# 10XGenomics/scan-rs

Hardware: AMD Instinct MI355X
Metric: cells/sec for top-50 PCA on 1000000x33000 @3% nnz; achieved HBM GB/s vs roofline (higher is better)
Workload: dtype f64

## Files before the change

### scan-rs_amd/csrc/capi.cpp

```cpp
#include <algorithm>
#include <cmath>
#include <vector>

#include "common.hpp"
#include "col_moments_plan.hpp"
#include "bk_plan.hpp"
#include "spmm_route.hpp"
#include "shard_exchange.hpp"

namespace scanrs {

static void allreduce_any(Storage &st, void *d, uint64_t count, int dtype) {
    if (!st.shard.active()) return;
    if (st.prof.on) st.prof.begin(st.stream, dtype == 0 ? "allreduce_f64" : "allreduce_u64", (double)count * 8.0);
    if (st.shard.comm) {
        comm_allreduce(st, st.shard.comm, d, count, dtype);
    } else if (st.shard.allreduce) {
        SCANRS_SYNC(st.stream);
        if (st.shard.allreduce(st.shard.ctx, d, count, dtype) != 0) fail(SCANRS_ERR_DEVICE, "all-reduce callback failed");
    } else {
        fail(SCANRS_ERR_ARGUMENT, "sharded handle without a transport");
    }
    if (st.prof.on) st.prof.end(st.stream);
}
// ... 1409 lines not shown
            st.device_factor = value != 0.0;
        } else if (k == "sseq_grid_cap") {
            st.sseq_grid_cap = as_u32(1, 16384);
        } else if (k == "merge_fused") {
            st.merge_fused = (int)as_u32(0, 1);
        } else if (k == "subset_scatter") {
            st.subset_scatter = (int)as_u32(0, 1);
        } else if (k == "d2h_threads") {
            st.d2h_threads = as_u32(1, 256);
        } else if (k == "sync_timeout_s") {
            set_sync_timeout_checked(value);
        } else if (k == "tile_spare_cus") {
            st.tile_spare_cus = value != 0.0;
        } else if (k == "tile_poison_slack") {
            st.tile_poison_slack = value != 0.0;
        } else if (k == "spmv_row_table") {
            st.spmv_row_table = value != 0.0;
        } else if (k == "gemm_direct") {
            st.gemm_direct = value != 0.0;
        } else if (k == "reuse_cmax") {
            if (!(value > 0.0)) fail(SCANRS_ERR_ARGUMENT, "reuse_cmax must be positive");
            st.reuse_cmax = value;
        } else {
            fail(SCANRS_ERR_ARGUMENT, "unknown option '%s'", key);
        }
    });
}
int scanrs_mat_get_counter(scanrs_mat *m, const char *key, uint64_t *value) {
    return guard([&] {
        if (!m || !key || !value) fail(SCANRS_ERR_ARGUMENT, "null argument");
// ... 17 lines not shown
                *value = d.flagged_older;
            else if (k == "bk_limit_branch")
                *value = d.limit_branch;
            else if (k == "bk_limit_bits")
                *value = bits(d.limit);
            else if (k == "bk_direct_columns")
                *value = d.direct_columns;
            else if (k == "bk_last_direct")
                *value = d.last_direct;
            else if (k == "bk_full_direct")
                *value = d.full_direct;
            else if (k == "bk_early_projections")
                *value = d.early_projections;
            else if (k == "bk_cmax_dense_bits")
                *value = bits(d.cmax_dense);
            else
                fail(SCANRS_ERR_ARGUMENT, "unknown counter '%s'", key);
        } else if (k == "spmm_route")
            *value = m->st->spmm.family;
        else if (k == "spmm_form")
            *value = m->st->spmm.form;
        else if (k == "spmm_chunks")
            *value = m->st->spmm.chunks;
        else if (k == "partition_rounds")
            *value = m->st->partition_rounds;
        else if (k == "partition_allreduces")
            *value = m->st->partition_allreduces;
        else if (k == "de_pairs_passes")
            *value = m->st->de_pairs_passes;
        else if (k == "de_pairs_literal")
            *value = m->st->de_pairs_literal;
        else if (k == "de_shard_tests")
            *value = m->st->de_shard_tests;
        else if (k == "de_shard_allreduces")
            *value = m->st->de_shard_allreduces;
        else if (k == "subset_masked_passes")
// ... 318 lines not shown
```

### scan-rs_amd/csrc/common.hpp

```cpp
#pragma once
#include <atomic>
#include <chrono>
#include <condition_variable>
#include <cstring>
#include <cstdio>
#include <cstdint>
#include <cstdarg>
#include <functional>
#include <map>
#include <set>
#include <memory>
#include <mutex>
#include <new>
#include <string>
#include <thread>
#include <utility>
#include <vector>

#include <hip/hip_runtime.h>

#include "scanrs_amd.h"
#include "common_err.hpp"

struct scanrs_comm;
// ... 326 lines not shown
    uint32_t sseq_grid_cap = 16384;
    int merge_fused = 1;
    size_t l2_tile_bytes = 3584u << 10;
    int spmm_order = 1;
    uint32_t hot_segment = 512;
    uint64_t blocked_min_nnz = 1ull << 22;
    int slice_walk = 1;
    int spmv_lds = 1;
    int dense_side_no_lds = 0;
    int overlap = 1;
    const int *skip_flag = nullptr;
    uint64_t orth_fallbacks = 0;
    uint64_t bk_host_retries = 0;
    struct BkDecisions {
        uint64_t q = 0, b = 0, coef_valid = 0, flagged_older = 0, limit_branch = 0, direct_columns = 0, last_direct = 0, full_direct = 0,
                 early_projections = 0;
        double limit = 0.0, cmax_dense = 0.0;
    } bk;
    int col_moments = 1;
    int device_factor = 1;
    unsigned d2h_threads = 4;
    int tile_poison_slack = 0;
    int tile_spare_cus = 1;
    int spmv_row_table = 1;
    int gemm_direct = 1;
    double reuse_cmax = 1e5;
    int materialize = 1;
    struct SpmmDecision {
        uint64_t family = 0, form = 0, chunks = 0;
    } spmm;
    ~Storage();
    SparseCopy &copy_with_outer_rows(bool outer_rows);
};
struct Storage::SideBuild {
    std::thread th;
    hipStream_t stream = nullptr;
    const SparseCopy *order[2] = {nullptr, nullptr};
    bool want_layout[2] = {false, false};
// ... 429 lines not shown
```

### scan-rs_amd/csrc/kernels.hip

```cpp
#include "common.hpp"
#include "device_map.hpp"
#include "spmm_route.hpp"
#include "launch_util.hpp"

#include <algorithm>
#include <rocprim/rocprim.hpp>

namespace scanrs {

template <typename T>
struct Vec2;
template <>
struct Vec2<double> {
    typedef d2 type;
};
template <>
struct Vec2<uint32_t> {
    typedef u2 type;
};

template <typename T>
__device__ __forceinline__ T bcast(T v, uint32_t lane);
template <>
__device__ __forceinline__ double bcast<double>(double v, uint32_t lane) {
// ... 1276 lines not shown
        hipLaunchKernelGGL((slab_reduce_kernel<double, 1>), dim3((cp.n_multi + 3u) / 4u), block, 0, st.stream, cp.multi.p, cp.n_multi,
                           slab, l, out, ldo, off_a, rank, off_w, ldw);
    SCANRS_HIP(hipGetLastError());
}

void launch_spmm_f64(Storage &st, SparseCopy &cp, const DevMap &map, const double *X, uint32_t ldx, uint32_t l,
                     double *out, uint32_t ldo, const double *off_a, uint32_t rank, const double *off_w, uint32_t ldw) {
    SpmmQuery q = spmm_query(st, cp, map, l, ldx);
    const bool tiles = tiles_static_candidate(q) && (path_forces_tiles(q.o) || spmm_tiles_auto(st, cp, map));
    SpmmRoute r = spmm_route(q, tiles);
    if (r.materialized && !fvals_room(cp)) {
        q.values_room = false;
        r = spmm_route(q, tiles);
    }
    st.spmm = {(uint64_t)r.family, r.form_bits(), r.chunk_bits()};
    if (r.even_ld && ((ldx & 1u) || (ldo & 1u))) fail(SCANRS_ERR_ARGUMENT, "panel leading dimensions must be even");
    const double *fv = r.materialized ? ensure_fvals(st, cp, map, r.fstart) : nullptr;
    switch (r.family) {
    case SPMM_TILES:
        for (uint32_t c0 = 0; c0 < l; c0 += r.chunk_width) {
            const uint32_t lw = std::min(r.chunk_width, l - c0);
            if (r.sliver && c0 + lw == l)
                launch_spmm_t<double>(st, cp, map, X + c0, ldx, lw, out + c0, ldo, off_a, rank, off_w ? off_w + c0 : nullptr, ldw);
            else
                launch_spmm_tiles(st, cp, map, X + c0, ldx, lw, out + c0, ldo, off_a, rank, off_w ? off_w + c0 : nullptr, ldw);
        }
        return;
    case SPMM_GATHER2D: return launch_spmm_2d(st, cp, map, X, ldx, l, out, ldo, off_a, rank, off_w, ldw);
    case SPMM_GATHER2D_F32: return launch_spmm_2d_f32(st, cp, map, X, ldx, l, out, ldo, off_a, rank, off_w, ldw);
    case SPMM_SLICE_WALK:
// ... 118 lines not shown
```

### scan-rs_amd/csrc/solver.cpp

```cpp
#include <algorithm>
#include <atomic>
#include <cmath>
#include <cstdlib>
#include <cstring>
#include <future>
#include <sys/mman.h>
#include <memory>
#include <mutex>
#include <thread>
#include <vector>

#include "bk_plan.hpp"
#include "common.hpp"
#include "host_team.hpp"

namespace scanrs {

struct SmallRng {
    uint64_t s[4];
    explicit SmallRng(uint64_t seed) {
        uint64_t state = seed;
        for (int i = 0; i < 4; i++) {
            state += 0x9E3779B97F4A7C15ull;
            uint64_t z = state;
// ... 1123 lines not shown
            for (uint32_t r = 0; r < q; r++)
                for (uint32_t j = 0; j < q; j++) colmax[j] = std::max(colmax[j], std::fabs(cfull[(size_t)r * q + j]));
        if (reuse && !c_valid && trace_on())
            fprintf(stderr, "[scanrs trace] bk: rank-deficient panels were completed on the host: the projection is computed directly\n");
        plan = bk_plan(colmax.data(), b, n_iter, c.st.reuse_cmax, c_valid);
        bk_record(c.st.bk, plan, c_valid);
        if (tracked && trace_on()) bk_plan_trace(colmax.data(), b, n_iter, plan);
        if (tracked && !plan.last_direct) {
            Tick tk("bk: last block product");
            mat_apply(m, to_t_transpose, P, ldb, b, T + (size_t)(n_iter - 1) * b, ldq);
        }
    }

    const double *project() {
        Tick tk("bk: projection");
        if (plan.full_direct) {
            wait_early_projections();
            mat_apply(m, to_t_transpose, K, ldq, q, T, ldq);
        } else {
            for (uint32_t j = n_iter - 1 - (plan.last_direct ? 1u : 0u); j >= 1; j--)
                if (!projected[j]) project_block(c, j, "bk_projw");
            if (!block0_copied) launch_copy_cols(c.st, T, ldq, T2, ldq, dt, b);
            wait_early_projections();
            if (!plan.direct.empty()) {
                const uint32_t nbad = (uint32_t)plan.direct.size(), ldbad = even_up(nbad);
                uint32_t *d_idx = c.st.scratch.get<uint32_t>("bk_badidx", nbad);
                SCANRS_HIP(hipMemcpyAsync(d_idx, plan.direct.data(), (size_t)nbad * 4, hipMemcpyHostToDevice, c.s));
                c.sync();
                double *Qbad = c.dev("bk_Qbad", (size_t)ds * ldbad);
                double *Tbad = c.dev("bk_Tbad", (size_t)dt * ldbad);
                launch_permute_cols(c.st, K, ldq, Qbad, ldbad, ds, d_idx, nbad, false);
                mat_apply(m, to_t_transpose, Qbad, ldbad, nbad, Tbad, ldbad);
                launch_permute_cols(c.st, Tbad, ldbad, T2, ldq, dt, d_idx, nbad, true);
            }
        }
        stage_mark("bk projection sync");
        c.sync();
        stage_mark("bk projection synced");
        return plan.full_direct ? T : T2;
// ... 285 lines not shown
```

### scan-rs_amd/csrc/tiles.hip

```cpp
#include "common.hpp"
#include "device_map.hpp"
#include "spmm_route.hpp"

#include <algorithm>
#include <rocprim/rocprim.hpp>

namespace scanrs {

namespace {

#ifndef TL_NW_DEF
#define TL_NW_DEF 8
#endif
constexpr uint32_t TL_NW = TL_NW_DEF;
constexpr int TL_W = 6;
#ifndef TL_SROWS
#define TL_SROWS 1
#endif
#ifndef TL_DPPW
#define TL_DPPW 1
#endif
typedef uint32_t u32x16 __attribute__((ext_vector_type(16)));
constexpr uint32_t TL_TABC = 8;

// ... 676 lines not shown
    DevBuf<double> uo, vi;
    DevBuf<double> uo_slot;
    DevBuf<double> ratio_tab;
    bool dense = false;
    uint32_t dn_wgg = 0, dn_items = 0;
    uint64_t dn_chunks = 0;
    uint64_t dn_served = 0;
    uint64_t src_nnz = 0;
    DevBuf<uint32_t> drec;
    DevBuf<uint64_t> cmeta;
    DevBuf<char> ditems;
    DevBuf<uint32_t> rtab;
    int slot_mode = 0;
    DevBuf<uint32_t> slot_order;
    DevBuf<uint32_t> slot_pos;
    DevBuf<double> w_place, w_inner;
    bool fold_inner = false, fold_outer = false;
    bool separable = false;
    int wsrc = 0;
    DevBuf<double> wtab;
    uint64_t wtab_stride = 0;
    int sig_n = -1;
    uint32_t sig_id[MAX_OPS] = {};
    int sig_outer[MAX_OPS] = {};
    double bytes() const {
        return (double)prow.n * 2.0 + (double)pcnt.n + (double)pw.n * 8.0 + (double)ov.nnz * 16.0 + (double)ratio_tab.n * 8.0 + (double)drec.n * 4.0 + (double)cmeta.n * 8.0 +
               (double)rtab.n * 4.0 + (double)wtab.n * 8.0 + (double)(w_place.n + w_inner.n) * 8.0;
    }
    bool structure_matches(const Storage &st) const {
        if (dense != tile_dense_wanted(st)) return false;
        if (dense && (slot_order.n != 0) != (st.tile_sort_slots != 0 && n_slots > 1)) return false;
        if (dense && slot_order.n != 0 && slot_mode != st.tile_sort_slots) return false;
        const bool splittable = default_tile_shape(spmm_options(st));
        const double want_x = splittable && st.tile_split ? st.tile_split_x : 0.0, want_min = splittable && st.tile_split ? st.tile_split_min : 0.0;
        return sh.K == st.tile_k && sh.S == st.tile_s && sh.T == st.tile_t && sh.B == st.tile_b && sh.KU == tile_unit_positions(spmm_options(st)) &&
               split_x == want_x && split_min == want_min;
    }
    bool weights_match(const DevMap &map) const {
        if (sig_n != map.n) return false;
        for (int i = 0; i < map.n; i++)
            if (sig_id[i] != map.ops[i].id || sig_outer[i] != map.ops[i].a_outer) return false;
        return true;
// ... 268 lines not shown
        } else
        hipLaunchKernelGGL(tile_weights_kernel, grid, dim3(256), 0, st.stream, tl.prow.p, tl.pcnt.p, tl.pw.p, n_rec,
                           tl.slot_vec.p, tl.n_slots, tl.sh, map, tl.unit_mode ? tl.uo.p : (const double *)nullptr, tl.unit_mode ? tl.vi.p : (const double *)nullptr, skip,
                           tl.unit_mode ? tl.ratio_tab.p : (const double *)nullptr, nl_outer, vmajor ? (uint32_t)tl.n_groups : 0u);
    }
    if (tl.ov.nnz) materialize_map_values(st, tl.ov, map, tl.ov.fvals.p);
    SCANRS_HIP(hipGetLastError());
    if (trace_on()) (void)wait_stream_quiet(st.stream);
    tl.sig_n = map.n;
    for (int i = 0; i < map.n; i++) {
        tl.sig_id[i] = map.ops[i].id;
        tl.sig_outer[i] = map.ops[i].a_outer;
    }
}

#include "tiles_dense.inc"

namespace {

struct TileArgs {
    const uint16_t *prow;
    const double *pw;
    const double *uo;
    uint32_t *next_item;
    uint64_t n_groups, n_outer, n_inner;
    TileShape sh;
};

template <int K, int S, int KU>
__device__ __forceinline__ void spmm_tile_body(const TileArgs &ta, const double *__restrict__ X, uint32_t ldx, uint32_t l,
// ... 217 lines not shown
                                                                  uint32_t n_items) {
    spmm_tile_body<K, S, KU>(ta, X, ldx, l, parts, ldo, part_stride, n_items);
}
template <int K, int S, int KU>
__global__ __launch_bounds__(64 * TL_NW) __attribute__((amdgpu_waves_per_eu(3, 3))) void spmm_tile_kernel_r168(
    TileArgs ta, const double *__restrict__ X, uint32_t ldx, uint32_t l, double *__restrict__ parts, uint32_t ldo, uint64_t part_stride,
    uint32_t n_items) {
    spmm_tile_body<K, S, KU>(ta, X, ldx, l, parts, ldo, part_stride, n_items);
}

__global__ __launch_bounds__(256) void tile_finish_kernel(const double *__restrict__ parts, uint32_t n_parts, uint64_t part_stride,
                                                          const uint32_t *__restrict__ slot_first, const uint32_t *__restrict__ slot_pos,
                                                          const double *__restrict__ ovout, uint64_t n_outer,
                                                          uint32_t l, uint32_t ldp, uint32_t ldo, double *__restrict__ out, const double *__restrict__ off_a,
                                                          uint32_t rank, const double *__restrict__ off_w, uint32_t ldw, const uint64_t *__restrict__ ov_indptr,
                                                          const double *__restrict__ uo) {
    const uint32_t hp = (l + 1u) / 2u;
    const uint64_t e = (uint64_t)blockIdx.x * blockDim.x + threadIdx.x;
    if (e >= n_outer * hp) return;
    const uint64_t o = e / hp;
    const uint32_t c = (uint32_t)(e % hp) * 2u;
    d2 s = (d2){0.0, 0.0};
    const uint32_t s0 = slot_first[o], s1 = slot_first[o + 1];
    for (uint32_t sl = s0; sl < s1; sl++) {
        const size_t at = slot_pos ? slot_pos[sl] : sl;
        d2 t = *reinterpret_cast<const d2 *>(parts + at * ldp + c);
        for (uint32_t p = 1; p < n_parts; p++) {
            const d2 u = *reinterpret_cast<const d2 *>(parts + (size_t)p * part_stride + at * ldp + c);
            t.x += u.x;
            t.y += u.y;
        }
        if (sl == s0) {
            s = t;
        } else {
            s.x += t.x;
            s.y += t.y;
        }
    }
    if (uo) {
        const double f = uo[o];
        s.x *= f;
        s.y *= f;
    }
    if (ovout && ov_indptr[o + 1] > ov_indptr[o]) {
        const d2 t = *reinterpret_cast<const d2 *>(ovout + o * ldp + c);
        s.x += t.x;
        s.y += t.y;
    }
    for (uint32_t q = 0; q < rank; q++) {
        const double aq = off_a[o * rank + q];
        s.x += aq * off_w[(size_t)q * ldw + c];
        if (c + 1 < l) s.y += aq * off_w[(size_t)q * ldw + c + 1];
    }
    *reinterpret_cast<d2 *>(out + o * ldo + c) = s;
}

template <int K, int S, int KU>
void launch_tile_kernel(Storage &st, const TileArgs &ta, const double *X, uint32_t ldx, uint32_t l, double *parts, uint32_t ldo,
                        uint64_t part_stride, uint32_t n_items, uint32_t grid) {
    const size_t shmem = ((size_t)ta.sh.B * ta.sh.T + 1u) * ldx * 8;
    if constexpr (S <= 28) {
        SCANRS_HIP(hipFuncSetAttribute((const void *)spmm_tile_kernel_r168<K, S, KU>, hipFuncAttributeMaxDynamicSharedMemorySize, (int)shmem));
        hipLaunchKernelGGL((spmm_tile_kernel_r168<K, S, KU>), dim3(grid), dim3(64 * TL_NW), shmem, st.stream, ta, X, ldx, l, parts, ldo, part_stride,
                           n_items);
    } else {
        SCANRS_HIP(hipFuncSetAttribute((const void *)spmm_tile_kernel<K, S, KU>, hipFuncAttributeMaxDynamicSharedMemorySize, (int)shmem));
        hipLaunchKernelGGL((spmm_tile_kernel<K, S, KU>), dim3(grid), dim3(64 * TL_NW), shmem, st.stream, ta, X, ldx, l, parts, ldo, part_stride,
                           n_items);
// ... 110 lines not shown
    const uint64_t part_stride = std::max<uint64_t>(tl.n_slots, 1) * (uint64_t)ldc;
    double *pbuf = st.scratch.get<double>("tile_parts", (size_t)sh.n_parts * part_stride);
    double *ovout = nullptr;
    if (tl.ov.nnz) {
        ovout = st.scratch.get<double>("tile_ovout", (size_t)cp.n_outer * ldc);
        if (st.tile_overlap) {
            hipStream_t ovs = st.ov();
            SCANRS_HIP(hipEventRecord(st.ev_in, st.stream));
            SCANRS_HIP(hipStreamWaitEvent(ovs, st.ev_in, 0));
            launch_gather2d_ov(st, ovs, tl.ov, Xov, Xov == X ? ldx : ldxov, l, ovout, ldc);
            SCANRS_HIP(hipEventRecord(st.ev_ov, ovs));
        } else {
            launch_gather2d_ov(st, st.stream, tl.ov, Xov, Xov == X ? ldx : ldxov, l, ovout, ldc);
        }
    }
    uint32_t *next_item = st.scratch.get<uint32_t>("tile_next_item", 1);
    SCANRS_HIP(hipMemsetAsync(next_item, 0, sizeof(uint32_t), st.stream));
    TileArgs ta{tl.prow.p, tl.pw.p, tl.unit_mode ? tl.uo_slot.p : nullptr, next_item, tl.n_groups, tl.n_slots, cp.n_inner, sh};
    const double bytes = (double)(cp.nnz - tl.ov.nnz) * 8.0 + (double)(cp.n_outer + 1) * 8.0 + (double)cp.n_inner * l * 8.0 + (double)cp.n_outer * l * 8.0;
    const bool long_outer = cp.n_outer >= cp.n_inner;
    if (st.prof.on)
        st.prof.begin(st.stream, long_outer ? "spmm_tile_kernel/long-outer" : "spmm_tile_kernel/short-outer", bytes,
                      tl.dense ? (double)tl.dn_served * 8.0 * l  : (double)tl.n_groups * sh.nt * sh.S * sh.K * 8.0 * l);
#define SCANRS_TILE(KK, SS, UU) launch_tile_kernel<KK, SS, UU>(st, ta, X, ldx, l, pbuf, ldc, part_stride, n_items, grid)
    const bool um = tl.unit_mode;
    if (n_items == 0) {
    } else if (tl.dense) {
        launch_tile_dense_kernel(st, tl, X, ldx, l, pbuf, ldc, part_stride, next_item, grid);
    } else if (sh.K == 2 && sh.S == 32)
        um ? SCANRS_TILE(2, 32, 1) : SCANRS_TILE(2, 32, 0);
    else if (sh.K == 2 && sh.S == 28)
        um ? SCANRS_TILE(2, 28, 1) : SCANRS_TILE(2, 28, 0);
    else if (sh.K == 3 && sh.S == 32)
        SCANRS_TILE(3, 32, 0);
    else if (sh.K == 4 && sh.S == 32)
        SCANRS_TILE(4, 32, 0);
    else if (sh.K == 4 && sh.S == 28)
        SCANRS_TILE(4, 28, 0);
    else
        fail(SCANRS_ERR_ARGUMENT, "unsupported tile shape K=%u S=%u", sh.K, sh.S);
#undef SCANRS_TILE
    if (st.prof.on) st.prof.end(st.stream);
    if (ovout && st.tile_overlap) SCANRS_HIP(hipStreamWaitEvent(st.stream, st.ev_ov, 0));
    const uint64_t n = cp.n_outer * (uint64_t)((l + 1u) / 2u);
    hipLaunchKernelGGL(tile_finish_kernel, dim3((unsigned)((n + 255) / 256)), dim3(256), 0, st.stream, pbuf, sh.n_parts, part_stride, tl.slot_first.p, tl.slot_pos.p, ovout,
                       cp.n_outer, l, ldc, ldo, out, off_a, rank, off_w, ldw, tl.ov.indptr.p, (tl.dense && tl.fold_outer) ? tl.uo.p : (const double *)nullptr);
    SCANRS_HIP(hipGetLastError());
}

double *tile_panel_copy_target(Storage &st, SparseCopy &cp, uint32_t l) {
    if ((l & 1u) || l < TL_LMIN || l > TL_LMAX || !cp.tiles || !cp.tiles->dense || cp.tiles->unit_mode || cp.tiles->fold_inner || !cp.tiles->structure_matches(st)) return nullptr;
    const SpmmOptions o = spmm_options(st);
    if (!(path_forces_tiles(o) || (path_auto(o) && o.tile_auto && f64_panels(o)))) return nullptr;
    return st.scratch.get<double>("tile_xc", ((size_t)cp.n_inner + 3u * cp.tiles->sh.T) * l);
}

__global__ void warm_tiles_kernel() {}
void warm_tiles(hipStream_t s) { hipLaunchKernelGGL(warm_tiles_kernel, dim3(1), dim3(64), 0, s); }

}
```

### scan-rs_amd/csrc/tiles_dense.inc

```

namespace {

typedef double d16 __attribute__((ext_vector_type(16)));

constexpr uint32_t DN_S = 32, DN_G = 16, DN_RC = 4;
constexpr uint32_t DN_NULL = (DN_B * DN_T) << 16;
constexpr uint32_t DN_PRE = 4;
constexpr uint32_t DN_FRONT = 8;
constexpr uint32_t DN_BACK = 8;

struct DenseBigList {
    unsigned long long *cursor;
    uint64_t *key;
    uint32_t *val;
    uint64_t cap;
};
template <int MODE>
__global__ __launch_bounds__(64) void dense_walk_kernel(const uint64_t *__restrict__ indptr, const uint32_t *__restrict__ indices,
                                                        const uint32_t *__restrict__ values, const uint32_t *__restrict__ slot_vec,
                                                        const uint32_t *__restrict__ slot_first, const uint32_t *__restrict__ slot_order, uint64_t n_slots,
                                                        uint64_t n_groups, TileShape sh, uint32_t *__restrict__ cnt, const uint64_t *__restrict__ off, uint32_t *__restrict__ sorted,
                                                        unsigned long long *__restrict__ ovc, const unsigned long long *__restrict__ ov_off,
                                                        unsigned long long *__restrict__ ov_cursor, uint32_t *__restrict__ ov_indices,
                                                        uint32_t *__restrict__ ov_values, DenseBigList big_list) {
// ... 374 lines not shown
    if (threadIdx.x == 0) {
        uint64_t want = 0;
        if (g < n_groups)
            for (uint32_t v = t0; v < t1; v++) want += cnt[g * sh.nt + v];
        if (want != n_real) {
            const unsigned long long k = atomicAdd(&bad[0], 1ull);
            if (k < 8) {
                bad[1 + 4 * k] = g;
                bad[2 + 4 * k] = part;
                bad[3 + 4 * k] = want;
                bad[4 + 4 * k] = n_real;
            }
        }
    }
}
__global__ void dense_fill_null_kernel(uint32_t *__restrict__ rec, uint64_t n) {
    const uint64_t i = (uint64_t)blockIdx.x * blockDim.x + threadIdx.x;
    if (i < n) rec[i] = DN_NULL;
}

__global__ void dense_place_tables_kernel(const uint32_t *__restrict__ slot_vec, const uint32_t *__restrict__ slot_order, uint64_t n_slots, const double *__restrict__ uo,
                                          const double *__restrict__ ratio, int tab_outer, double *__restrict__ fpl, double *__restrict__ tabp) {
    const uint64_t i = (uint64_t)blockIdx.x * blockDim.x + threadIdx.x;
    const uint64_t place = tab_outer ? i / TL_TABC : i;
    if (place >= n_slots) return;
    const uint32_t outer = slot_vec[slot_order ? slot_order[place] : place];
    if (tab_outer)
        tabp[i] = uo[outer] * ratio[(size_t)outer * TL_TABC + (i - place * TL_TABC)];
    else
        fpl[place] = uo[outer];
// ... 145 lines not shown
#ifdef SCANRS_DENSE_STAMPS
#define SCANRS_DENSE_CLOBBERS "memory", "scc", "vcc", "m0", "s2", "s3", "s4", "s5", "s6", "s7", "s8", "s9", "s10", "s11", "s12", "s13", "s14", "s15", "s16", "s17", "s18", "s19", "s20", "s21", "s22", "s23", "s24", "s25", "s26", "s27", "s28", "s29", "s30", "s31", "s32", "s33", "s34", "s35", "s36", "s37", "s38", "s39", "s40", "s41", "s42", "s43", "s44", "s45", "s46", "s47", "s48", "s49", "s50", "s51", "s52", "s53", "s54", "s55", "s56", "s57", "s58", "s59", "s60", "s61", "s62", "s63", "s64", "s65", "s66", "s67", "s68", "s69", "s70", "s71", "s72", "s73", "s74", "s75", "s76", "s77", "s78", "s79", "s80", "s81", "s82", "s83", "s84", "s85", "s86", "s87", "s88", "s89", "s90", "s91", "s92", "s93", "s94", "s95", "s96", "s97", "s98", "s99", "s100", "s101", "v26", "v27", "v28", "v29", "v30", "v31", "v32", "v33", "v34", "v35", "v36", "v37", "v38", "v39", "v40", "v41", "v42", "v43", "v44", "v45", "v46", "v47", "v48", "v49", "v50", "v51", "v52", "v53", "v54", "v55", "v56", "v57", "v58", "v59", "v60", "v61", "v62", "v63", "v64", "v65", "v66", "v67", "v68", "v69", "v70", "v71", "v72", "v73", "v74", "v75", "v76", "v77", "v78", "v79", "v80", "v81", "v82", "v83", "v84", "v85", "v86", "v87"
#else
#define SCANRS_DENSE_CLOBBERS "memory", "scc", "vcc", "m0", "s12", "s13", "s14", "s15", "s16", "s17", "s18", "s19", "s20", "s21", "s22", "s23", "s24", "s25", "s26", "s27", "s28", "s29", "s30", "s31", "s32", "s33", "s34", "s35", "s36", "s37", "s38", "s39", "s40", "s41", "s42", "s43", "s44", "s45", "s46", "s47", "s48", "s49", "s50", "s51", "s52", "s53", "s54", "s55", "s56", "s57", "s58", "s59", "s60", "s61", "s62", "s63", "s64", "s65", "s66", "s67", "s68", "s69", "s70", "s71", "s72", "s73", "s74", "s75", "s76", "s77", "s78", "s79", "s80", "s81", "s82", "s83", "s84", "s85", "s86", "s87", "s88", "s89", "s90", "s91", "s92", "s93", "s94", "s95", "s96", "s97", "s98", "s99", "s100", "s101", "v26", "v27", "v28", "v29", "v30", "v31", "v32", "v33", "v34", "v35", "v36", "v37", "v38", "v39", "v40", "v41", "v42", "v43", "v44", "v45", "v46", "v47", "v48", "v49", "v50", "v51", "v52", "v53", "v54", "v55", "v56", "v57", "v58", "v59", "v60", "v61", "v62", "v63", "v64", "v65", "v66", "v67", "v68", "v69", "v70", "v71", "v72", "v73", "v74", "v75", "v76", "v77", "v78", "v79", "v80", "v81", "v82", "v83", "v84", "v85", "v86", "v87"
#endif

#define SCANRS_DENSE_COMMON_OPERANDS                                                                                                                              \
    [reclo] "v"((uint32_t)(uintptr_t)recp), [rechi] "v"((uint32_t)((uintptr_t)recp >> 32)), [rtablo] "v"((uint32_t)(uintptr_t)rtab),                         \
        [rtabhi] "v"((uint32_t)((uintptr_t)rtab >> 32)), [srclo] "v"((uint32_t)(uintptr_t)src), [srchi] "v"((uint32_t)((uintptr_t)src >> 32)),               \
        [nrounds] "v"(it.n_rounds), [wave10] "v"(wave * 1024u), [lds0] "v"(lds0), [lane4] "v"(lane * 4u), [ring] "v"(ring), [rowb] "v"(rowbytes)
#ifdef SCANRS_DENSE_STAMPS
#define SCANRS_DENSE_STAMP_OPERANDS [stamplo] "v"((uint32_t)(uintptr_t)da.stamps), [stamphi] "v"((uint32_t)((uintptr_t)da.stamps >> 32)),
#else
#define SCANRS_DENSE_STAMP_OPERANDS
#endif
template <int WSRC>
__global__ __launch_bounds__(64 * TL_NW, 2) __attribute__((amdgpu_num_vgpr(216))) void spmm_tile_dense_kernel(DenseArgs da, const double *__restrict__ X, uint32_t ldx, uint32_t l,
                                                                        double *__restrict__ parts, uint32_t ldo, uint64_t part_stride, uint32_t n_items) {
    extern __shared__ __attribute__((aligned(16))) char lds[];
    const uint32_t lane = threadIdx.x & 63u, wave = (uint32_t)__builtin_amdgcn_readfirstlane((int)(threadIdx.x >> 6));
    const uint32_t rowbytes = ldx * 8u;
    const uint32_t tile_bytes = DN_T * rowbytes;
    const char *Xb = reinterpret_cast<const char *>(X);
    const uint32_t lds0 = (uint32_t)(uintptr_t)(lds_ptr_t)lds;
    {
        const uint32_t zoff = DN_B * tile_bytes;
        for (uint32_t i = threadIdx.x * 16u; i < rowbytes; i += blockDim.x * 16u) *reinterpret_cast<d2 *>(lds + zoff + i) = (d2){0.0, 0.0};
    }
    constexpr int CH = 5;
    uint32_t voff[CH];
#pragma unroll
    for (int i = 0; i < CH; i++) voff[i] = min((wave + (uint32_t)i * TL_NW) * 1024u, tile_bytes - 1024u) + lane * 16u;
    uint32_t src_lane = lane;
// ... 25 lines not shown
        {
            const uint32_t base = lds0 + (t0 & 3u) * tile_bytes;
            const char *sbase = Xb + (uint64_t)t0 * tile_bytes;
#pragma unroll
            for (int i = 0; i < CH; i++) {
                const uint32_t coff = min((wave + (uint32_t)i * TL_NW) * 1024u, tile_bytes - 1024u);
                asm volatile("s_add_u32 m0, %0, %1\n\ts_nop 0\n\tglobal_load_lds_dwordx4 %2, %3" ::"s"(base), "s"(coff), "v"(voff[i]), "s"(sbase) : "memory", "scc");
            }
        }
        d16 a0 = 0.0, a1 = 0.0, a2 = 0.0, a3 = 0.0;
        const uint64_t chunk0 = (uint64_t)it.rec_base + (uint64_t)wave * it.cpw;
        const uint32_t *recp = da.rec + chunk0 * DN_G;
        const uint32_t *rtab = da.rtab + it.round_base;
        const char *src = Xb + (uint64_t)t0 * tile_bytes;
        if constexpr (WSRC == 0) {
            const double *pwp = da.pw + chunk0 * DN_G + (lane & 15u);
            const uint32_t dst = lds0 + (t0 & 3u) * tile_bytes;
            const uint32_t pwlo = (uint32_t)(uintptr_t)pwp, pwhi = (uint32_t)((uintptr_t)pwp >> 32);
            asm volatile(
#include "tile_dense_body.inc"
                : "+{v[88:119]}"(a0), "+{v[120:151]}"(a1), "+{v[152:183]}"(a2), "+{v[184:215]}"(a3)
                : SCANRS_DENSE_STAMP_OPERANDS SCANRS_DENSE_COMMON_OPERANDS, [dst] "v"(dst), [pwlo] "v"(pwlo), [pwhi] "v"(pwhi)
                : SCANRS_DENSE_CLOBBERS);
        } else if constexpr (WSRC == 1) {
            const double *tabp = da.tab + group * (uint64_t)(DN_S * DN_TABK);
            asm volatile(
#include "tile_dense_body_tabo.inc"
                : "+{v[88:119]}"(a0), "+{v[120:151]}"(a1), "+{v[152:183]}"(a2), "+{v[184:215]}"(a3)
                : SCANRS_DENSE_STAMP_OPERANDS SCANRS_DENSE_COMMON_OPERANDS, [t0] "v"(t0), [tablo] "v"((uint32_t)(uintptr_t)tabp), [tabhi] "v"((uint32_t)((uintptr_t)tabp >> 32))
                : SCANRS_DENSE_CLOBBERS);
        } else {
            asm volatile(
#include "tile_dense_body_tabi.inc"
                : "+{v[88:119]}"(a0), "+{v[120:151]}"(a1), "+{v[152:183]}"(a2), "+{v[184:215]}"(a3)
                : SCANRS_DENSE_STAMP_OPERANDS SCANRS_DENSE_COMMON_OPERANDS, [t0] "v"(t0), [tablo] "v"((uint32_t)(uintptr_t)da.tab), [tabhi] "v"((uint32_t)((uintptr_t)da.tab >> 32)),
                  [stride8] "v"(da.tab_stride8)
                : SCANRS_DENSE_CLOBBERS);
        }
        if (live && lane * 2u < l) {
            double *dstp = parts + (size_t)part * part_stride;
            const d16 *acc[4] = {&a0, &a1, &a2, &a3};
#pragma unroll
            for (int sl = 0; sl < (int)DN_S; sl++) {
                const uint64_t o = group * DN_S + sl;
                if (o < da.n_slots) {
                    const d16 &t = *acc[sl / 8];
                    *reinterpret_cast<d2 *>(dstp + o * ldo + lane * 2u) = (d2){t[(sl % 8) * 2], t[(sl % 8) * 2 + 1]};
                }
            }
        }
    }
}

}

static TileLayout *dense_layout_build(Storage &st, const SparseCopy &cp, double max_overflow, hipStream_t s, std::unique_ptr<TileLayout> tl,
                                      const std::function<void(const char *)> &lap) {
    TileShape &sh = tl->sh;
    const bool split = tl->split_x > 0.0;
    const uint64_t n_seg = cp.n_outer * sh.n_parts;
    const uint32_t n_wgg = (uint32_t)((tl->n_groups + TL_NW - 1) / TL_NW);
    const uint64_t n_items64 = (uint64_t)n_wgg * sh.n_parts;
// ... 209 lines not shown
        DevBuf<uint32_t> ki(n_ov), vi2(n_ov);
        unsigned end_bit = 1;
        while (end_bit < 32u && (cp.n_inner >> end_bit) != 0) end_bit++;
        const SplitSegment seg_begin{ov.indptr.p, tl->slot_first.p, 0}, seg_end{ov.indptr.p, tl->slot_first.p, 1};
        auto it_b = rocprim::make_transform_iterator(rocprim::make_counting_iterator<unsigned>(0u), seg_begin);
        auto it_e = rocprim::make_transform_iterator(rocprim::make_counting_iterator<unsigned>(0u), seg_end);
        size_t tb = 0;
        SCANRS_HIP(rocprim::segmented_radix_sort_pairs(nullptr, tb, ov.indices.p, ki.p, ov.values.p, vi2.p, (unsigned)n_ov, (unsigned)cp.n_outer, it_b, it_e, 0u, end_bit, s));
        DevBuf<char> tsort(std::max<size_t>(tb, 16));
        SCANRS_HIP(rocprim::segmented_radix_sort_pairs(tsort.p, tb, ov.indices.p, ki.p, ov.values.p, vi2.p, (unsigned)n_ov, (unsigned)cp.n_outer, it_b, it_e, 0u, end_bit, s));
        hipLaunchKernelGGL(tile_split_copyback_kernel, grid_1d(cp.n_outer), dim3(256), 0, s, ov.indptr.p, tl->slot_first.p, cp.n_outer, ki.p, vi2.p, ov.indices.p,
                           ov.values.p);
        SCANRS_SYNC(s);
        lap("overflow sort");
    }
    if (n_ov) ensure_bounds(st, ov, s);
    SCANRS_SYNC(s);
    lap("overflow bounds");
    if (trace_on())
        fprintf(stderr, "[scanrs trace] dense tile layout: %llu outer x %llu inner, %llu slots (most per vector %u) in %llu groups x %u tiles in %u parts = %u items, nnz %llu, "
                        "overflow %llu (%.2f %%), positions per served nonzero %.3f, rounds per visit %.2f, %.2f GB\n",
                (unsigned long long)cp.n_outer, (unsigned long long)cp.n_inner, (unsigned long long)tl->n_slots, tl->max_mult, (unsigned long long)tl->n_groups, sh.nt,
                sh.n_parts, n_items, (unsigned long long)cp.nnz, (unsigned long long)n_ov, 100.0 * (double)n_ov / (double)std::max<uint64_t>(1, cp.nnz),
                (double)(n_chunks - DN_FRONT) * DN_G / (double)std::max<uint64_t>(1, n_served), (double)tot_rounds / std::max<double>(1.0, (double)n_wgg * (sh.nt + sh.n_parts)),
                tl->bytes() / 1e9);
    return tl.release();
}

static void dense_layout_weights(Storage &st, TileLayout &tl, const SparseCopy &cp, const DevMap &map) {
    const int nl_outer = tile_layout_set_form(st, tl, cp, map).nl_outer;
// ... 41 lines not shown
                           tl.slot_vec.p, tl.slot_order.p, tl.n_slots, cp.n_inner, map, tl.separable ? 1 : 0, nl_outer, tl.w_place.p, tl.w_place.p,
                           nl_outer ? (const double *)nullptr : tl.w_inner.p, tl.vi.p, fold ? 1 : 0);
        if (st.prof.on) st.prof.end(st.stream);
    }
    if (tl.ov.nnz) materialize_map_values(st, tl.ov, map, tl.ov.fvals.p);
    SCANRS_HIP(hipGetLastError());
    if (trace_on()) (void)wait_stream_quiet(st.stream);
    tl.sig_n = map.n;
    for (int i = 0; i < map.n; i++) {
        tl.sig_id[i] = map.ops[i].id;
        tl.sig_outer[i] = map.ops[i].a_outer;
    }
}

static void launch_tile_dense_kernel(Storage &st, const TileLayout &tl, const double *X, uint32_t ldx, uint32_t l, double *parts, uint32_t ldo, uint64_t part_stride,
                                     uint32_t *next_item, uint32_t grid) {
    static const bool want_stamps = getenv("SCANRS_DENSE_STAMPS") != nullptr;
    uint32_t *stamps = st.scratch.get<uint32_t>("tile_stamps", 32);
    if (want_stamps) SCANRS_HIP(hipMemsetAsync(stamps, 0, 32 * 4, st.stream));
    DenseArgs da{tl.drec.p, tl.pw.p, tl.wsrc == 2 ? tl.wtab.p + DN_TABI_FRONT : tl.wtab.p, (uint32_t)(tl.wtab_stride * 8u), reinterpret_cast<const DenseItem *>(tl.ditems.p), tl.rtab.p, next_item,
                 tl.n_groups, tl.n_slots, tl.dn_wgg, tl.sh.tpp, tl.sh.nt, stamps};
    const size_t shmem = (size_t)DN_B * DN_T * ldx * 8 + 1024 + TL_NW * 256;
#define SCANRS_DENSE_LAUNCH(W)                                                                                                                                   \
    do {                                                                                                                                                         \
        SCANRS_HIP(hipFuncSetAttribute((const void *)spmm_tile_dense_kernel<W>, hipFuncAttributeMaxDynamicSharedMemorySize, (int)shmem));                        \
        hipLaunchKernelGGL(spmm_tile_dense_kernel<W>, dim3(grid), dim3(64 * TL_NW), shmem, st.stream, da, X, ldx, l, parts, ldo, part_stride, tl.dn_items);       \
    } while (0)
    if (tl.wsrc == 1)
        SCANRS_DENSE_LAUNCH(1);
    else if (tl.wsrc == 2)
        SCANRS_DENSE_LAUNCH(2);
    else
        SCANRS_DENSE_LAUNCH(0);
#undef SCANRS_DENSE_LAUNCH
    if (want_stamps) {
        unsigned long long h[12] = {0, 0, 0, 0, 0, 0, 0, 0, 0, 0, 0, 0};
        SCANRS_D2H(h, stamps, sizeof(h), st.stream);
        if (h[3])
            fprintf(stderr, "[scanrs stamps] %llu wave-rounds: body %.0f clk, wait for staging / weights / scalar loads %.0f clk, barrier %.0f clk per round\n", h[3],
                    (double)h[0] / h[3], (double)h[1] / h[3], (double)h[2] / h[3]);
        if (h[3]) {
// ... 7 lines not shown
```

Before: 5.010 million.

## Write single-slot rows directly from dense tile kernel and project contiguous BK columns in place

Rows covered by exactly one slot with no overflow are now finished (scale, low-rank offset) inside the dense tile kernel and written straight to the output. The finish kernel then runs only over a precomputed list of remaining rows. This removes a round trip through the partial buffer for most rows. Separately, when the BK direct-projection columns form an even-aligned contiguous range, they are projected in place instead of through a gather/scatter with an uploaded index list. The cost is a one-time mark/scan setup, extra scalar loads and branching in the dense kernel's epilogue, and some register pressure risk.

New measurement: 5.054 million (median of 6 runs). Within noise of the previous version (+0.9%).

```diff
diff --git a/scan-rs_amd/csrc/capi.cpp b/scan-rs_amd/csrc/capi.cpp
--- a/scan-rs_amd/csrc/capi.cpp
+++ b/scan-rs_amd/csrc/capi.cpp
@@ -1447,6 +1447,10 @@
             st.tile_spare_cus = value != 0.0;
         } else if (k == "tile_poison_slack") {
             st.tile_poison_slack = value != 0.0;
+        } else if (k == "tile_direct_rows") {
+            st.tile_direct_rows = value != 0.0;
+        } else if (k == "bk_direct_in_place") {
+            st.bk_direct_in_place = value != 0.0;
         } else if (k == "spmv_row_table") {
             st.spmv_row_table = value != 0.0;
         } else if (k == "gemm_direct") {
@@ -1494,12 +1498,16 @@
                 *value = d.early_projections;
             else if (k == "bk_cmax_dense_bits")
                 *value = bits(d.cmax_dense);
+            else if (k == "bk_direct_in_place")
+                *value = d.direct_in_place;
             else
                 fail(SCANRS_ERR_ARGUMENT, "unknown counter '%s'", key);
         } else if (k == "spmm_route")
             *value = m->st->spmm.family;
         else if (k == "spmm_form")
             *value = m->st->spmm.form;
+        else if (k == "tile_direct_rows")
+            *value = m->st->tile_direct_rows_last;
         else if (k == "spmm_chunks")
             *value = m->st->spmm.chunks;
         else if (k == "partition_rounds")
diff --git a/scan-rs_amd/csrc/common.hpp b/scan-rs_amd/csrc/common.hpp
--- a/scan-rs_amd/csrc/common.hpp
+++ b/scan-rs_amd/csrc/common.hpp
@@ -364,7 +364,7 @@
     uint64_t bk_host_retries = 0;
     struct BkDecisions {
         uint64_t q = 0, b = 0, coef_valid = 0, flagged_older = 0, limit_branch = 0, direct_columns = 0, last_direct = 0, full_direct = 0,
-                 early_projections = 0;
+                 early_projections = 0, direct_in_place = 0;
         double limit = 0.0, cmax_dense = 0.0;
     } bk;
     int col_moments = 1;
@@ -372,6 +372,9 @@
     unsigned d2h_threads = 4;
     int tile_poison_slack = 0;
     int tile_spare_cus = 1;
+    int tile_direct_rows = 1;
+    uint64_t tile_direct_rows_last = 0;
+    int bk_direct_in_place = 1;
     int spmv_row_table = 1;
     int gemm_direct = 1;
     double reuse_cmax = 1e5;
diff --git a/scan-rs_amd/csrc/kernels.hip b/scan-rs_amd/csrc/kernels.hip
--- a/scan-rs_amd/csrc/kernels.hip
+++ b/scan-rs_amd/csrc/kernels.hip
@@ -1314,6 +1314,7 @@
         r = spmm_route(q, tiles);
     }
     st.spmm = {(uint64_t)r.family, r.form_bits(), r.chunk_bits()};
+    st.tile_direct_rows_last = 0;
     if (r.even_ld && ((ldx & 1u) || (ldo & 1u))) fail(SCANRS_ERR_ARGUMENT, "panel leading dimensions must be even");
     const double *fv = r.materialized ? ensure_fvals(st, cp, map, r.fstart) : nullptr;
     switch (r.family) {
diff --git a/scan-rs_amd/csrc/solver.cpp b/scan-rs_amd/csrc/solver.cpp
--- a/scan-rs_amd/csrc/solver.cpp
+++ b/scan-rs_amd/csrc/solver.cpp
@@ -1161,6 +1161,7 @@
 
     const double *project() {
         Tick tk("bk: projection");
+        c.st.bk.direct_in_place = 0;
         if (plan.full_direct) {
             wait_early_projections();
             mat_apply(m, to_t_transpose, K, ldq, q, T, ldq);
@@ -1169,7 +1170,13 @@
                 if (!projected[j]) project_block(c, j, "bk_projw");
             if (!block0_copied) launch_copy_cols(c.st, T, ldq, T2, ldq, dt, b);
             wait_early_projections();
-            if (!plan.direct.empty()) {
+            bool run = c.st.bk_direct_in_place && !plan.direct.empty() && plan.direct.front() % 2u == 0u && plan.direct.size() % 2u == 0u;
+            for (size_t i = 1; run && i < plan.direct.size(); i++) run = plan.direct[i] == plan.direct[0] + (uint32_t)i;
+            c.st.bk.direct_in_place = run;
+            if (run) {
+                const uint32_t first = plan.direct.front(), nbad = (uint32_t)plan.direct.size();
+                mat_apply(m, to_t_transpose, K + first, ldq, nbad, T2 + first, ldq);
+            } else if (!plan.direct.empty()) {
                 const uint32_t nbad = (uint32_t)plan.direct.size(), ldbad = even_up(nbad);
                 uint32_t *d_idx = c.st.scratch.get<uint32_t>("bk_badidx", nbad);
                 SCANRS_HIP(hipMemcpyAsync(d_idx, plan.direct.data(), (size_t)nbad * 4, hipMemcpyHostToDevice, c.s));
diff --git a/scan-rs_amd/csrc/tiles.hip b/scan-rs_amd/csrc/tiles.hip
--- a/scan-rs_amd/csrc/tiles.hip
+++ b/scan-rs_amd/csrc/tiles.hip
@@ -714,6 +714,9 @@
     int slot_mode = 0;
     DevBuf<uint32_t> slot_order;
     DevBuf<uint32_t> slot_pos;
+    DevBuf<uint32_t> place_vec;
+    DevBuf<uint32_t> rest_list;
+    uint64_t n_direct = 0, n_rest = 0;
     DevBuf<double> w_place, w_inner;
     bool fold_inner = false, fold_outer = false;
     bool separable = false;
@@ -725,7 +728,7 @@
     int sig_outer[MAX_OPS] = {};
     double bytes() const {
         return (double)prow.n * 2.0 + (double)pcnt.n + (double)pw.n * 8.0 + (double)ov.nnz * 16.0 + (double)ratio_tab.n * 8.0 + (double)drec.n * 4.0 + (double)cmeta.n * 8.0 +
-               (double)rtab.n * 4.0 + (double)wtab.n * 8.0 + (double)(w_place.n + w_inner.n) * 8.0;
+               (double)rtab.n * 4.0 + (double)wtab.n * 8.0 + (double)(w_place.n + w_inner.n) * 8.0 + (double)(place_vec.n + rest_list.n) * 4.0;
     }
     bool structure_matches(const Storage &st) const {
         if (dense != tile_dense_wanted(st)) return false;
@@ -1024,6 +1027,29 @@
     }
 }
 
+template <typename P>
+__device__ __forceinline__ void tile_finish_scale(d2 &s, uint64_t o, P uo) {
+    if (uo) {
+        const double f = uo[o];
+        s.x *= f;
+        s.y *= f;
+    }
+}
+template <typename P>
+__device__ __forceinline__ void tile_finish_offset(d2 &s, uint64_t o, uint32_t c, uint32_t l, P off_a, uint32_t rank, P off_w, uint32_t ldw) {
+    for (uint32_t q = 0; q < rank; q++) {
+        const double aq = off_a[o * rank + q];
+        const P wq = off_w + (size_t)q * ldw;
+        s.x += aq * wq[c];
+        if (c + 1 < l) s.y += aq * wq[c + 1];
+    }
+}
+template <typename P>
+__device__ __forceinline__ void tile_finish_row(d2 &s, uint64_t o, uint32_t c, uint32_t l, P uo, P off_a, uint32_t rank, P off_w, uint32_t ldw) {
+    tile_finish_scale(s, o, uo);
+    tile_finish_offset(s, o, c, l, off_a, rank, off_w, ldw);
+}
+
 #include "tiles_dense.inc"
 
 namespace {
@@ -1271,11 +1297,11 @@
                                                           const double *__restrict__ ovout, uint64_t n_outer,
                                                           uint32_t l, uint32_t ldp, uint32_t ldo, double *__restrict__ out, const double *__restrict__ off_a,
                                                           uint32_t rank, const double *__restrict__ off_w, uint32_t ldw, const uint64_t *__restrict__ ov_indptr,
-                                                          const double *__restrict__ uo) {
+                                                          const double *__restrict__ uo, const uint32_t *__restrict__ list) {
     const uint32_t hp = (l + 1u) / 2u;
     const uint64_t e = (uint64_t)blockIdx.x * blockDim.x + threadIdx.x;
     if (e >= n_outer * hp) return;
-    const uint64_t o = e / hp;
+    const uint64_t o = list ? (uint64_t)list[e / hp] : e / hp;
     const uint32_t c = (uint32_t)(e % hp) * 2u;
     d2 s = (d2){0.0, 0.0};
     const uint32_t s0 = slot_first[o], s1 = slot_first[o + 1];
@@ -1294,21 +1320,13 @@
             s.y += t.y;
         }
     }
-    if (uo) {
-        const double f = uo[o];
-        s.x *= f;
-        s.y *= f;
-    }
+    tile_finish_scale(s, o, uo);
     if (ovout && ov_indptr[o + 1] > ov_indptr[o]) {
         const d2 t = *reinterpret_cast<const d2 *>(ovout + o * ldp + c);
         s.x += t.x;
         s.y += t.y;
     }
-    for (uint32_t q = 0; q < rank; q++) {
-        const double aq = off_a[o * rank + q];
-        s.x += aq * off_w[(size_t)q * ldw + c];
-        if (c + 1 < l) s.y += aq * off_w[(size_t)q * ldw + c + 1];
-    }
+    tile_finish_offset(s, o, c, l, off_a, rank, off_w, ldw);
     *reinterpret_cast<d2 *>(out + o * ldo + c) = s;
 }
 
@@ -1449,8 +1467,17 @@
             launch_gather2d_ov(st, st.stream, tl.ov, Xov, Xov == X ? ldx : ldxov, l, ovout, ldc);
         }
     }
+    const double *uo_fin = (tl.dense && tl.fold_outer) ? tl.uo.p : (const double *)nullptr;
+    const bool direct = tl.dense && st.tile_direct_rows && n_items != 0 && sh.n_parts == 1u && tl.place_vec.n != 0;
+    st.tile_direct_rows_last = direct ? tl.n_direct : 0;
     uint32_t *next_item = st.scratch.get<uint32_t>("tile_next_item", 1);
-    SCANRS_HIP(hipMemsetAsync(next_item, 0, sizeof(uint32_t), st.stream));
+    DenseDirect *dd_dev = nullptr;
+    if (direct) {
+        dd_dev = reinterpret_cast<DenseDirect *>(st.scratch.get<double>("tile_direct_args", sizeof(DenseDirect) / 8));
+        hipLaunchKernelGGL(dense_prepare_kernel, dim3(1), dim3(64), 0, st.stream, next_item, dd_dev, DenseDirect{tl.place_vec.p, out, uo_fin, off_a, off_w, ldo, rank, ldw, {0u, 0u, 0u}});
+    } else {
+        SCANRS_HIP(hipMemsetAsync(next_item, 0, sizeof(uint32_t), st.stream));
+    }
     TileArgs ta{tl.prow.p, tl.pw.p, tl.unit_mode ? tl.uo_slot.p : nullptr, next_item, tl.n_groups, tl.n_slots, cp.n_inner, sh};
     const double bytes = (double)(cp.nnz - tl.ov.nnz) * 8.0 + (double)(cp.n_outer + 1) * 8.0 + (double)cp.n_inner * l * 8.0 + (double)cp.n_outer * l * 8.0;
     const bool long_outer = cp.n_outer >= cp.n_inner;
@@ -1461,7 +1488,7 @@
     const bool um = tl.unit_mode;
     if (n_items == 0) {
     } else if (tl.dense) {
-        launch_tile_dense_kernel(st, tl, X, ldx, l, pbuf, ldc, part_stride, next_item, grid);
+        launch_tile_dense_kernel(st, tl, X, ldx, l, pbuf, ldc, part_stride, next_item, grid, dd_dev);
     } else if (sh.K == 2 && sh.S == 32)
         um ? SCANRS_TILE(2, 32, 1) : SCANRS_TILE(2, 32, 0);
     else if (sh.K == 2 && sh.S == 28)
@@ -1477,9 +1504,11 @@
 #undef SCANRS_TILE
     if (st.prof.on) st.prof.end(st.stream);
     if (ovout && st.tile_overlap) SCANRS_HIP(hipStreamWaitEvent(st.stream, st.ev_ov, 0));
-    const uint64_t n = cp.n_outer * (uint64_t)((l + 1u) / 2u);
-    hipLaunchKernelGGL(tile_finish_kernel, dim3((unsigned)((n + 255) / 256)), dim3(256), 0, st.stream, pbuf, sh.n_parts, part_stride, tl.slot_first.p, tl.slot_pos.p, ovout,
-                       cp.n_outer, l, ldc, ldo, out, off_a, rank, off_w, ldw, tl.ov.indptr.p, (tl.dense && tl.fold_outer) ? tl.uo.p : (const double *)nullptr);
+    const uint64_t n_fin = direct ? tl.n_rest : cp.n_outer;
+    const uint64_t n = n_fin * (uint64_t)((l + 1u) / 2u);
+    if (n)
+        hipLaunchKernelGGL(tile_finish_kernel, dim3((unsigned)((n + 255) / 256)), dim3(256), 0, st.stream, pbuf, sh.n_parts, part_stride, tl.slot_first.p, tl.slot_pos.p, ovout,
+                           n_fin, l, ldc, ldo, out, off_a, rank, off_w, ldw, tl.ov.indptr.p, uo_fin, direct ? tl.rest_list.p : (const uint32_t *)nullptr);
     SCANRS_HIP(hipGetLastError());
 }
 
diff --git a/scan-rs_amd/csrc/tiles_dense.inc b/scan-rs_amd/csrc/tiles_dense.inc
--- a/scan-rs_amd/csrc/tiles_dense.inc
+++ b/scan-rs_amd/csrc/tiles_dense.inc
@@ -412,6 +412,23 @@
         }
     }
 }
+__global__ void dense_direct_mark_kernel(const uint64_t *__restrict__ indptr, const uint32_t *__restrict__ slot_first, const uint32_t *__restrict__ slot_pos,
+                                         const uint64_t *__restrict__ ov_indptr, uint64_t n_outer, uint32_t *__restrict__ place_vec, uint32_t *__restrict__ flag) {
+    const uint64_t o = (uint64_t)blockIdx.x * blockDim.x + threadIdx.x;
+    if (o > n_outer) return;
+    if (o == n_outer) {
+        flag[o] = 0u;
+        return;
+    }
+    const uint32_t s0 = slot_first[o];
+    const bool direct = slot_first[o + 1] - s0 == 1u && ov_indptr[o + 1] == ov_indptr[o] && indptr[o + 1] > indptr[o];
+    if (direct) place_vec[slot_pos ? slot_pos[s0] : s0] = (uint32_t)o;
+    flag[o] = direct ? 0u : 1u;
+}
+__global__ void dense_direct_list_kernel(const uint32_t *__restrict__ flag, const uint32_t *__restrict__ pos, uint64_t n_outer, uint32_t *__restrict__ list) {
+    const uint64_t o = (uint64_t)blockIdx.x * blockDim.x + threadIdx.x;
+    if (o < n_outer && flag[o]) list[pos[o]] = (uint32_t)o;
+}
 __global__ void dense_fill_null_kernel(uint32_t *__restrict__ rec, uint64_t n) {
     const uint64_t i = (uint64_t)blockIdx.x * blockDim.x + threadIdx.x;
     if (i < n) rec[i] = DN_NULL;
@@ -587,9 +604,34 @@
 #else
 #define SCANRS_DENSE_STAMP_OPERANDS
 #endif
+constexpr uint32_t DN_NOT_DIRECT = 0xFFFFFFFFu;
+struct DenseDirect {
+    const uint32_t *place_vec;
+    double *out;
+    const double *uo, *off_a, *off_w;
+    uint32_t ldo, rank, ldw;
+    uint32_t pad[3];
+};
+static_assert(sizeof(DenseDirect) == 64 && offsetof(DenseDirect, ldo) == 40, "spmm_tile_dense_kernel reads DenseDirect by word");
+__global__ void dense_prepare_kernel(uint32_t *__restrict__ next_item, DenseDirect *__restrict__ dst, DenseDirect dd) {
+    if (threadIdx.x == 0) {
+        *next_item = 0u;
+        if (dst) *dst = dd;
+    }
+}
+typedef const __attribute__((address_space(1))) double *gcd_t;
+typedef __attribute__((address_space(1))) double *gd_t;
+typedef uint32_t gu4 __attribute__((ext_vector_type(4)));
+__device__ __forceinline__ uint32_t dn_uniform(uint32_t x) { return (uint32_t)__builtin_amdgcn_readfirstlane((int)x); }
+template <typename T>
+__device__ __forceinline__ T *dn_uniform(T *p) {
+    const uint64_t u = (uint64_t)(uintptr_t)p;
+    return reinterpret_cast<T *>((uintptr_t)(((uint64_t)dn_uniform((uint32_t)(u >> 32)) << 32) | dn_uniform((uint32_t)u)));
+}
 template <int WSRC>
 __global__ __launch_bounds__(64 * TL_NW, 2) __attribute__((amdgpu_num_vgpr(216))) void spmm_tile_dense_kernel(DenseArgs da, const double *__restrict__ X, uint32_t ldx, uint32_t l,
-                                                                        double *__restrict__ parts, uint32_t ldo, uint64_t part_stride, uint32_t n_items) {
+                                                                        double *__restrict__ parts, uint32_t ldo, uint64_t part_stride, uint32_t n_items,
+                                                                        const DenseDirect *ddp) {
     extern __shared__ __attribute__((aligned(16))) char lds[];
     const uint32_t lane = threadIdx.x & 63u, wave = (uint32_t)__builtin_amdgcn_readfirstlane((int)(threadIdx.x >> 6));
     const uint32_t rowbytes = ldx * 8u;
@@ -645,7 +687,9 @@
         const uint32_t *rtab = da.rtab + it.round_base;
         const char *src = Xb + (uint64_t)t0 * tile_bytes;
         if constexpr (WSRC == 0) {
-            const double *pwp = da.pw + chunk0 * DN_G + (lane & 15u);
+            uint32_t lw = lane;
+            asm volatile("" : "+v"(lw));
+            const double *pwp = da.pw + chunk0 * DN_G + (lw & 15u);
             const uint32_t dst = lds0 + (t0 & 3u) * tile_bytes;
             const uint32_t pwlo = (uint32_t)(uintptr_t)pwp, pwhi = (uint32_t)((uintptr_t)pwp >> 32);
             asm volatile(
@@ -671,12 +715,58 @@
         if (live && lane * 2u < l) {
             double *dstp = parts + (size_t)part * part_stride;
             const d16 *acc[4] = {&a0, &a1, &a2, &a3};
-#pragma unroll
-            for (int sl = 0; sl < (int)DN_S; sl++) {
-                const uint64_t o = group * DN_S + sl;
-                if (o < da.n_slots) {
-                    const d16 &t = *acc[sl / 8];
-                    *reinterpret_cast<d2 *>(dstp + o * ldo + lane * 2u) = (d2){t[(sl % 8) * 2], t[(sl % 8) * 2 + 1]};
+            uint32_t ln = lane;
+            asm volatile("" : "+v"(ln));
+            uint32_t w[16];
+#pragma unroll
+            for (int k = 0; k < 4; k++) {
+                if (ddp) {
+                    const gu4 q = reinterpret_cast<const __attribute__((address_space(1))) gu4 *>((const __attribute__((address_space(1))) char *)ddp)[k];
+                    w[4 * k] = dn_uniform(q.x), w[4 * k + 1] = dn_uniform(q.y), w[4 * k + 2] = dn_uniform(q.z), w[4 * k + 3] = dn_uniform(q.w);
+                } else {
+                    w[4 * k] = w[4 * k + 1] = w[4 * k + 2] = w[4 * k + 3] = 0u;
+                }
+                __builtin_amdgcn_sched_barrier(0);
+            }
+            auto ptr_of = [&](int i) { return (uintptr_t)(((uint64_t)w[2 * i + 1] << 32) | w[2 * i]); };
+            DenseDirect dd;
+            dd.place_vec = reinterpret_cast<const uint32_t *>(ptr_of(0));
+            dd.out = reinterpret_cast<double *>(ptr_of(1));
+            dd.uo = reinterpret_cast<const double *>(ptr_of(2));
+            dd.off_a = reinterpret_cast<const double *>(ptr_of(3));
+            dd.off_w = reinterpret_cast<const double *>(ptr_of(4));
+            dd.ldo = w[10], dd.rank = w[11], dd.ldw = w[12];
+#pragma unroll
+            for (int q8 = 0; q8 < (int)DN_S / 8; q8++) {
+                uint32_t vecs[8];
+                __builtin_amdgcn_sched_barrier(0);
+                if (dd.place_vec) {
+                    const uint32_t mine = ((const __attribute__((address_space(1))) uint32_t *)dd.place_vec)[group * DN_S + (uint32_t)q8 * 8u + (ln & 7u)];
+#pragma unroll
+                    for (int i = 0; i < 8; i++) vecs[i] = (uint32_t)__builtin_amdgcn_readlane((int)mine, i);
+                } else {
+#pragma unroll
+                    for (int i = 0; i < 8; i++) vecs[i] = DN_NOT_DIRECT;
+                }
+                __builtin_amdgcn_sched_barrier(0);
+#pragma unroll
+                for (int i = 0; i < 8; i++) {
+                    const int sl = q8 * 8 + i;
+                    const uint64_t o = group * DN_S + sl;
+                    if (o < da.n_slots) {
+                        const d16 &t = *acc[q8];
+                        d2 s = (d2){t[i * 2], t[i * 2 + 1]};
+                        const uint32_t vec = vecs[i];
+                        if (vec != DN_NOT_DIRECT) {
+                            tile_finish_row(s, vec, ln * 2u, l, (gcd_t)dd.uo, (gcd_t)dd.off_a, dd.rank, (gcd_t)dd.off_w, dd.ldw);
+                            const gd_t row = (gd_t)dd.out + (size_t)vec * dd.ldo;
+                            *reinterpret_cast<__attribute__((address_space(1))) d2 *>(row + ln * 2u) = s;
+                        } else {
+                            double *row = dstp + o * ldo;
+                            *reinterpret_cast<d2 *>(row + ln * 2u) = s;
+                        }
+                    }
+                    __builtin_amdgcn_sched_barrier(0);
                 }
             }
         }
@@ -916,6 +1006,25 @@
         SCANRS_SYNC(s);
         lap("overflow sort");
     }
+    if (sh.n_parts == 1u && n_items) {
+        const uint64_t n_places = (uint64_t)n_wgg * TL_NW * DN_S;
+        tl->place_vec.alloc(n_places);
+        SCANRS_HIP(hipMemsetAsync(tl->place_vec.p, 0xFF, n_places * 4, s));
+        DevBuf<uint32_t> flag(cp.n_outer + 1), pos(cp.n_outer + 1);
+        hipLaunchKernelGGL(dense_direct_mark_kernel, grid_1d(cp.n_outer + 1), dim3(256), 0, s, cp.indptr.p, tl->slot_first.p, tl->slot_pos.p, ov.indptr.p, cp.n_outer,
+                           tl->place_vec.p, flag.p);
+        size_t tb = 0;
+        SCANRS_HIP(rocprim::exclusive_scan(nullptr, tb, flag.p, pos.p, 0u, (size_t)cp.n_outer + 1, rocprim::plus<uint32_t>(), s));
+        DevBuf<char> tmp(std::max<size_t>(tb, 16));
+        SCANRS_HIP(rocprim::exclusive_scan(tmp.p, tb, flag.p, pos.p, 0u, (size_t)cp.n_outer + 1, rocprim::plus<uint32_t>(), s));
+        const uint32_t n_rest = SCANRS_D2H_VALUE(pos.p + cp.n_outer, s);
+        tl->n_rest = n_rest;
+        tl->n_direct = cp.n_outer - n_rest;
+        tl->rest_list.alloc(std::max<uint32_t>(n_rest, 1));
+        if (n_rest) hipLaunchKernelGGL(dense_direct_list_kernel, grid_1d(cp.n_outer), dim3(256), 0, s, flag.p, pos.p, cp.n_outer, tl->rest_list.p);
+        SCANRS_SYNC(s);
+        lap("direct rows");
+    }
     if (n_ov) ensure_bounds(st, ov, s);
     SCANRS_SYNC(s);
     lap("overflow bounds");
@@ -987,7 +1096,7 @@
 }
 
 static void launch_tile_dense_kernel(Storage &st, const TileLayout &tl, const double *X, uint32_t ldx, uint32_t l, double *parts, uint32_t ldo, uint64_t part_stride,
-                                     uint32_t *next_item, uint32_t grid) {
+                                     uint32_t *next_item, uint32_t grid, const DenseDirect *dd) {
     static const bool want_stamps = getenv("SCANRS_DENSE_STAMPS") != nullptr;
     uint32_t *stamps = st.scratch.get<uint32_t>("tile_stamps", 32);
     if (want_stamps) SCANRS_HIP(hipMemsetAsync(stamps, 0, 32 * 4, st.stream));
@@ -997,7 +1106,7 @@
 #define SCANRS_DENSE_LAUNCH(W)                                                                                                                                   \
     do {                                                                                                                                                         \
         SCANRS_HIP(hipFuncSetAttribute((const void *)spmm_tile_dense_kernel<W>, hipFuncAttributeMaxDynamicSharedMemorySize, (int)shmem));                        \
-        hipLaunchKernelGGL(spmm_tile_dense_kernel<W>, dim3(grid), dim3(64 * TL_NW), shmem, st.stream, da, X, ldx, l, parts, ldo, part_stride, tl.dn_items);       \
+        hipLaunchKernelGGL(spmm_tile_dense_kernel<W>, dim3(grid), dim3(64 * TL_NW), shmem, st.stream, da, X, ldx, l, parts, ldo, part_stride, tl.dn_items, dd);   \
     } while (0)
     if (tl.wsrc == 1)
         SCANRS_DENSE_LAUNCH(1);
```
